# r9y9/deepvoice3_pytorch

Measured on NVIDIA H100. Metric: mel-frames/sec training step (B=16,T_mel=800), higher is better.
Workload: dtype f32 via split 16-bit pairs (fp16 pairs forward, bf16 pairs for gradients; 3 wgmma passes per product, fp32 accumulate)

## Files before the change

### deepvoice3_pytorch_b200/csrc/tc_gemm.cu

```cuda
#include "tc_common.cuh"
#include "../../include/dv3b200.h"

namespace dv3 {

using namespace tc;

constexpr int TC_CONV_THREADS = 512;
constexpr int TC_PRODUCER_REGS = 24;
constexpr int TC_CONSUMER_REGS = 176;
constexpr int TC_EPILOGUE_REGS = 136;
static_assert(TC_PRODUCER_REGS <= 65536 / TC_CONV_THREADS && TC_CONSUMER_REGS >= 65536 / TC_CONV_THREADS &&
              TC_EPILOGUE_REGS >= 65536 / TC_CONV_THREADS, "setmaxnreg direction of each warpgroup");
static_assert(128 * TC_PRODUCER_REGS + 256 * TC_CONSUMER_REGS + 128 * TC_EPILOGUE_REGS <= 65536, "register file");
constexpr int TC_WGRAD_THREADS = 288;
constexpr int MAX_TAPS_TC = 8;
constexpr int SMEM_LIMIT = 232448;
constexpr int RING_RESERVE = 32768;

enum { TC_GATED = 0, TC_CONV = 1 };

struct TcMaps { CUtensorMap a[2]; CUtensorMap b[2]; };

struct TcParams {
    int T, B;
    int Kc;
    int Nc;
    int rows_per_tap;
    int k, kb_n;
    int tap_off[MAX_TAPS_TC];
    const float* bias; const float* spk; const float* res;
    float* y; float* save_a; float* save_s;
    int gate_mode, residual;
    float* out; const float* e1; const float* e2; float alpha; int addmode, relu;
    float p_drop; const unsigned long long* seed_ptr; uint32_t salt;
    float gmain;
    int operand_bf16;
};

template <int BK> struct SwizzleOf;
template <> struct SwizzleOf<64> { static constexpr uint32_t layout = WG_SW128, sbo = 1024; };
template <> struct SwizzleOf<32> { static constexpr uint32_t layout = WG_SW64, sbo = 512; };

template <int BK>
__device__ __forceinline__ uint64_t make_desc(uint32_t saddr) {
    return make_wgmma_desc(saddr, 16, SwizzleOf<BK>::sbo, SwizzleOf<BK>::layout);
}

template <int NBOX, int BK, int BR, int NPL = 2>
struct TcCfg {
    static constexpr int TILE = 128 * BK * 2;
    static constexpr int TILE_B = BR * BK * 2;
    static constexpr int STAGE = NPL * (TILE + NBOX * TILE_B);
    static constexpr int NCOLS = BR * NBOX;
    static constexpr int ACC_PITCH = NCOLS + 1;
    static constexpr int ACC_TILE = 128 * ACC_PITCH * 4;
    static constexpr int STAGES_RAW = (SMEM_LIMIT - 2048 - RING_RESERVE - ACC_TILE) / STAGE;
    static constexpr int STAGES = STAGES_RAW > 6 ? 6 : STAGES_RAW;
    static constexpr int SMEM = STAGES * STAGE + ACC_TILE + 1024 + 512;
};
static_assert(TcCfg<2, 32, 64>::STAGES == 4, "gated forward: 4-stage ring");
static_assert(TcCfg<1, 32, 128>::STAGES == 4, "128-column conv: 4-stage ring");
static_assert(TcCfg<1, 64, 64>::STAGES == 3, "64-column conv at BK = 64: 3-stage ring");
static_assert(TcCfg<1, 32, 64>::STAGES == 6, "64-column conv at BK = 32: 6-stage ring");
static_assert(TcCfg<2, 64, 64, 1>::STAGES == 4, "single-pass gated forward: 4-stage ring");
static_assert(TcCfg<1, 64, 128, 1>::STAGES == 4, "single-pass 128-column conv at BK = 64: 4-stage ring");
static_assert(TcCfg<1, 32, 128, 1>::STAGES == 6, "single-pass 128-column conv at BK = 32: 6-stage ring");
static_assert(TcCfg<1, 64, 64, 1>::STAGES == 6, "single-pass 64-column conv at BK = 64: 6-stage ring");
static_assert(TcCfg<1, 32, 64, 1>::STAGES == 6, "single-pass 64-column conv at BK = 32: 6-stage ring");

template <int BR>
__device__ __forceinline__ void epilogue_gated(const TcParams& p, const float* arow, uint64_t* acc_empty, int a_row0,
                                               int a_z, int b_row0) {
    const int t = a_row0 + (threadIdx.x & 127), b = a_z, C = p.Nc;
    const bool tv = t < p.T;
    const float* __restrict__ bias = p.bias;
    const float* __restrict__ res = p.res;
    const float* __restrict__ spk = p.spk;
    float* __restrict__ yo = p.y;
    float* __restrict__ ao = p.save_a;
    float* __restrict__ so = p.save_s;
    const bool need_res = (p.gate_mode != 0) || p.residual;
    const size_t base = ((size_t)b * C + b_row0) * p.T + (tv ? t : 0);
#pragma unroll
    for (int c32 = 0; c32 < BR; c32 += 32) {
        float rr[32], sp[32];
        if (tv) {
            const size_t cb = base + (size_t)c32 * p.T;
#pragma unroll
            for (int i = 0; i < 32; ++i) rr[i] = need_res ? __ldg(&res[cb + (size_t)i * p.T]) : 0.f;
            if (spk) {
#pragma unroll
                for (int i = 0; i < 32; ++i) sp[i] = __ldg(&spk[cb + (size_t)i * p.T]);
            }
#pragma unroll
            for (int i = 0; i < 32; ++i) {
                const int c = b_row0 + c32 + i;
                const size_t idx = cb + (size_t)i * p.T;
                float va = arow[c32 + i];
                if (spk) va += sp[i];
                const float a = va + __ldg(&bias[c]);
                const float s = sigmoidf_(arow[BR + c32 + i] + __ldg(&bias[C + c]));
                float y;
                if (p.gate_mode == 0) {
                    y = a * s;
                    if (p.residual) y = (y + rr[i]) * 0.70710678118654752f;
                } else {
                    y = s * a + (1.f - s) * rr[i];
                }
                yo[idx] = y;
                if (ao) ao[idx] = a;
                if (so) so[idx] = s;
            }
        }
        if (c32 + 32 == BR) mbar_arrive(acc_empty);
    }
}

template <int NCOLS>
__device__ __forceinline__ void epilogue_conv(const TcParams& p, const float* arow, uint64_t* acc_empty, int a_row0,
                                              int a_z, int b_row0) {
    const int t = a_row0 + (threadIdx.x & 127), b = a_z;
    const bool tv = t < p.T;
    const DropCfg drop = make_drop(p.p_drop, p.seed_ptr, p.salt);
    const float* __restrict__ bias = p.bias;
    const float* __restrict__ e1 = p.e1;
    const float* __restrict__ e2 = p.e2;
    float* __restrict__ out = p.out;
#pragma unroll 1
    for (int c32 = 0; c32 < NCOLS; c32 += 32) {
        float v[32], x2[32];
        const int n0 = b_row0 + c32;
        const size_t cb = ((size_t)b * p.Nc + n0) * p.T + (tv ? t : 0);
        if (tv) {
#pragma unroll
            for (int i = 0; i < 32; ++i) {
                const bool ok = n0 + i < p.Nc;
                v[i] = (p.addmode != 0 && ok) ? __ldg(&e1[cb + (size_t)i * p.T]) : 0.f;
                x2[i] = (p.addmode == 2 && ok) ? __ldg(&e2[cb + (size_t)i * p.T]) : 0.f;
            }
#pragma unroll
            for (int i = 0; i < 32; ++i) {
                const int n = n0 + i;
                if (n < p.Nc) {
                    const size_t idx = cb + (size_t)i * p.T;
                    float g = arow[c32 + i] * drop_scale(drop, (uint32_t)idx);
                    if (bias) g += __ldg(&bias[n]);
                    if (p.addmode == 1) g += p.alpha * v[i];
                    else if (p.addmode == 2) g += v[i] * (1.f - x2[i]);
                    if (p.relu) g = fmaxf(g, 0.f);
                    out[idx] = g;
                }
            }
        }
        if (c32 + 32 == NCOLS) mbar_arrive(acc_empty);
    }
}

template <int MODE, int NBOX, int BR, int BK, bool BF16, int NPL>
__global__ void __launch_bounds__(TC_CONV_THREADS, 1)
tc_conv_kernel(const __grid_constant__ TcMaps maps, const __grid_constant__ TcParams p, int tiles_x, int tiles_y,
               int num_tiles) {
    pdl_trigger();
    static_assert(NPL == 1 || NPL == 2, "one or two operand planes");
    using Cfg = TcCfg<NBOX, BK, BR, NPL>;
    constexpr int TILE = Cfg::TILE, TILE_B = Cfg::TILE_B, STAGE = Cfg::STAGE, STAGES = Cfg::STAGES, NCOLS = Cfg::NCOLS;
    constexpr int B_OFF = NPL * TILE;
    constexpr int NR = NCOLS / 2;
    constexpr int A_HALF = 64 * BK * 2;
    static_assert(NCOLS <= 128, "main + cross accumulators must fit in the registers of a consumer thread");
    static_assert(STAGES >= 2, "pipeline needs at least two stages");
    extern __shared__ uint8_t smem_raw[];
    uint8_t* smem = reinterpret_cast<uint8_t*>((reinterpret_cast<uintptr_t>(smem_raw) + 1023) & ~(uintptr_t)1023);
    float* acc_tile = reinterpret_cast<float*>(smem + STAGES * STAGE);
    uint64_t* full = reinterpret_cast<uint64_t*>(smem + STAGES * STAGE + Cfg::ACC_TILE);
    uint64_t* empty = full + STAGES;
    uint64_t* acc_full = empty + STAGES;
    uint64_t* acc_empty = acc_full + 1;
    const int warp = threadIdx.x >> 5, lane = threadIdx.x & 31;
    const int n_iters = p.k * p.kb_n;

    if (threadIdx.x == 0) {
#pragma unroll
        for (int pl = 0; pl < NPL; ++pl) prefetch_tmap(&maps.a[pl]);
#pragma unroll
        for (int pl = 0; pl < NPL; ++pl) prefetch_tmap(&maps.b[pl]);
        for (int s = 0; s < STAGES; ++s) { mbar_init(&full[s], 1); mbar_init(&empty[s], 2); }
        mbar_init(acc_full, 256);
        mbar_init(acc_empty, 128);
        fence_barrier_init();
    }
    __syncthreads();
    pdl_wait();

    auto decode = [&](int tile, int& a_row0, int& a_z, int& b_row0, int& b_row1) {
        const int ty = tile % tiles_y, r = tile / tiles_y;
        const int tx = r % tiles_x;
        a_z = r / tiles_x;
        a_row0 = tx * 128;
        if (MODE == TC_GATED) { b_row0 = ty * BR; b_row1 = p.Nc + ty * BR; }
        else { b_row0 = ty * BR * NBOX; b_row1 = b_row0 + BR; }
    };

    if (warp >= 12) {
        setmaxnreg_inc<TC_EPILOGUE_REGS>();
        const float* arow = acc_tile + (threadIdx.x & 127) * Cfg::ACC_PITCH;
        int n = 0;
        for (int tile = blockIdx.x; tile < num_tiles; tile += gridDim.x, ++n) {
            int a_row0, a_z, b_row0, b_row1;
            decode(tile, a_row0, a_z, b_row0, b_row1);
            mbar_wait(acc_full, n & 1);
            if (MODE == TC_GATED) epilogue_gated<BR>(p, arow, acc_empty, a_row0, a_z, b_row0);
            else epilogue_conv<NCOLS>(p, arow, acc_empty, a_row0, a_z, b_row0);
        }
    } else if (warp >= 8) {
        setmaxnreg_dec<TC_PRODUCER_REGS>();
        if (warp == 8 && lane == 0) {
            int it = 0;
            for (int tile = blockIdx.x; tile < num_tiles; tile += gridDim.x) {
                int a_row0, a_z, b_row0, b_row1;
                decode(tile, a_row0, a_z, b_row0, b_row1);
                for (int kit = 0; kit < n_iters; ++kit, ++it) {
                    const int s = it % STAGES, ph = (it / STAGES) & 1;
                    mbar_wait(&empty[s], ph ^ 1);
                    uint8_t* st = smem + s * STAGE;
                    const int j = kit / p.kb_n, kb = kit - j * p.kb_n;
                    const int ax = kb * BK, ay = a_row0 + p.tap_off[j];
                    const int by0 = j * p.rows_per_tap + b_row0, by1 = j * p.rows_per_tap + b_row1;
                    mbar_arrive_expect_tx(&full[s], STAGE);
#pragma unroll
                    for (int pl = 0; pl < NPL; ++pl) {
                        tma_load_3d(st + pl * TILE, &maps.a[pl], &full[s], ax, ay, a_z);
                        uint8_t* bdst = st + B_OFF + pl * NBOX * TILE_B;
                        tma_load_3d(bdst, &maps.b[pl], &full[s], ax, by0, 0);
                        if (NBOX == 2) tma_load_3d(bdst + TILE_B, &maps.b[pl], &full[s], ax, by1, 0);
                    }
                }
            }
        }
    } else {
        setmaxnreg_inc<TC_CONSUMER_REGS>();
        const int wg = warp >> 2, wq = warp & 3;
        float acc[NR], xacc[NPL == 2 ? NR : 1];
        int it = 0, n = 0;
        for (int tile = blockIdx.x; tile < num_tiles; tile += gridDim.x, ++n) {
            int a_row0, a_z, b_row0, b_row1;
            decode(tile, a_row0, a_z, b_row0, b_row1);
#pragma unroll
            for (int i = 0; i < NR; ++i) {
                acc[i] = 0.f;
                if constexpr (NPL == 2) xacc[i] = 0.f;
            }
            for (int kit = 0; kit < n_iters; ++kit, ++it) {
                const int s = it % STAGES, ph = (it / STAGES) & 1;
                mbar_wait(&full[s], ph);
                const uint32_t sa = smem_u32(smem + s * STAGE) + wg * A_HALF;
                const uint32_t sb = smem_u32(smem + s * STAGE + B_OFF);
                wgmma_fence();
#pragma unroll
                for (int kk = 0; kk < BK / 16; ++kk) {
                    const uint32_t ko = kk * 32;
                    const uint64_t a0 = make_desc<BK>(sa + ko), b0 = make_desc<BK>(sb + ko);
                    wgmma_mma<NCOLS, 0, 0>(BF16, acc, a0, b0, 1);
                    if constexpr (NPL == 2) {
                        const uint64_t a1 = make_desc<BK>(sa + TILE + ko), b1 = make_desc<BK>(sb + NBOX * TILE_B + ko);
                        wgmma_mma<NCOLS, 0, 0>(BF16, xacc, a0, b1, 1);
                        wgmma_mma<NCOLS, 0, 0>(BF16, xacc, a1, b0, 1);
                    }
                }
                wgmma_commit();
                wgmma_wait<1>();
                if (kit > 0 && (threadIdx.x & 127) == 0) mbar_arrive(&empty[(it - 1) % STAGES]);
            }
            wgmma_wait<0>();
            if (n_iters > 0 && (threadIdx.x & 127) == 0) mbar_arrive(&empty[(it - 1) % STAGES]);
            mbar_wait(acc_empty, (n & 1) ^ 1);
#pragma unroll
            for (int i = 0; i < NR; ++i) {
                float* dst = &acc_tile[(64 * wg + frag_row(i, wq, lane)) * Cfg::ACC_PITCH + frag_col(i, lane)];
                if constexpr (NPL == 2) *dst = fmaf(xacc[i], LO_INV, acc[i] * p.gmain);
                else *dst = acc[i] * p.gmain;
            }
            mbar_arrive(acc_full);
        }
    }
}

struct TcMnParams {
    int T, B, Mw, Nw, k;
    int tap_off[MAX_TAPS_TC];
    int nsplit, batches_per_split, kb_n;
    float* dw; long long split_stride;
    int msplit; long long s_m, s_mh, s_n, s_j;
    float gcoef;
};

constexpr int WG_BOX = 64 * 32 * 2;
template <int NPL>
struct WgCfg {
    static constexpr int STAGE = NPL * (2 * WG_BOX + 2 * WG_BOX);
    static constexpr int STAGES = ((SMEM_LIMIT - 2048) / STAGE) > 6 ? 6 : ((SMEM_LIMIT - 2048) / STAGE);
    static constexpr int SMEM = STAGES * STAGE + 1024 + 512;
};
static_assert(WgCfg<2>::STAGES == 6 && WgCfg<1>::STAGES == 6, "weight gradient: 6-stage ring");

template <int NPL>
__global__ void __launch_bounds__(TC_WGRAD_THREADS, 1)
tc_wgrad_mn_kernel(const __grid_constant__ TcMaps maps, const __grid_constant__ TcMnParams p) {
    pdl_trigger();
    static_assert(NPL == 1 || NPL == 2, "one or two operand planes");
    constexpr int WG_STAGE = WgCfg<NPL>::STAGE, WG_STAGES = WgCfg<NPL>::STAGES;
    constexpr int A_PL = 2 * WG_BOX, B_PL = 2 * WG_BOX;
    constexpr uint32_t LBO = 4096, SBO = 1024;
    extern __shared__ uint8_t smem_raw[];
    uint8_t* smem = reinterpret_cast<uint8_t*>((reinterpret_cast<uintptr_t>(smem_raw) + 1023) & ~(uintptr_t)1023);
    uint64_t* full = reinterpret_cast<uint64_t*>(smem + WG_STAGES * WG_STAGE);
    uint64_t* empty = full + WG_STAGES;
    const int warp = threadIdx.x >> 5, lane = threadIdx.x & 31;

    const int wg_j = blockIdx.z % p.k, wg_split = blockIdx.z / p.k;
    const int m0 = blockIdx.y * 128, n0 = blockIdx.x * 128;
    const int b_beg = wg_split * p.batches_per_split;
    int b_end = b_beg + p.batches_per_split; if (b_end > p.B) b_end = p.B;
    const int n_iters = (b_end > b_beg ? b_end - b_beg : 0) * p.kb_n;

    if (threadIdx.x == 0) {
#pragma unroll
        for (int pl = 0; pl < NPL; ++pl) prefetch_tmap(&maps.a[pl]);
#pragma unroll
        for (int pl = 0; pl < NPL; ++pl) prefetch_tmap(&maps.b[pl]);
        for (int s = 0; s < WG_STAGES; ++s) { mbar_init(&full[s], 1); mbar_init(&empty[s], 2); }
        fence_barrier_init();
    }
    __syncthreads();
    pdl_wait();

    if (warp == 8) {
        if (lane == 0) {
            for (int it = 0; it < n_iters; ++it) {
                const int s = it % WG_STAGES, ph = (it / WG_STAGES) & 1;
                mbar_wait(&empty[s], ph ^ 1);
                uint8_t* st = smem + s * WG_STAGE;
                const int bi = it / p.kb_n, tc_ = it - bi * p.kb_n;
                const int b = b_beg + bi, t0 = tc_ * 32;
                mbar_arrive_expect_tx(&full[s], WG_STAGE);
#pragma unroll
                for (int pl = 0; pl < NPL; ++pl) {
#pragma unroll
                    for (int h = 0; h < 2; ++h)
                        tma_load_3d(st + pl * A_PL + h * WG_BOX, &maps.a[pl], &full[s], m0 + h * 64, t0, b);
#pragma unroll
                    for (int q = 0; q < 2; ++q)
                        tma_load_3d(st + NPL * A_PL + pl * B_PL + q * WG_BOX, &maps.b[pl], &full[s], n0 + q * 64,
                                    t0 + p.tap_off[wg_j], b);
                }
            }
        }
    } else {
        const int wg = warp >> 2, wq = warp & 3;
        float acc[NPL * 64];
#pragma unroll
        for (int i = 0; i < NPL * 64; ++i) acc[i] = 0.f;
        for (int it = 0; it < n_iters; ++it) {
            const int s = it % WG_STAGES, ph = (it / WG_STAGES) & 1;
            mbar_wait(&full[s], ph);
            const uint32_t sa = smem_u32(smem + s * WG_STAGE);
            wgmma_fence();
#pragma unroll
            for (int kk = 0; kk < 2; ++kk) {
                const uint32_t ko = kk * 16 * 128;
                const uint64_t a0 = make_wgmma_desc(sa + wg * WG_BOX + ko, LBO, SBO, WG_SW128);
                const uint64_t b0 = make_wgmma_desc(sa + NPL * A_PL + ko, LBO, SBO, WG_SW128);
                wgmma_mma<128, 1, 1>(true, acc, a0, b0, 1);
                if constexpr (NPL == 2) {
                    const uint64_t a1 = make_wgmma_desc(sa + A_PL + wg * WG_BOX + ko, LBO, SBO, WG_SW128);
                    const uint64_t b1 = make_wgmma_desc(sa + 2 * A_PL + B_PL + ko, LBO, SBO, WG_SW128);
                    wgmma_mma<128, 1, 1>(true, acc + 64, a0, b1, 1);
                    wgmma_mma<128, 1, 1>(true, acc + 64, a1, b0, 1);
                }
            }
            wgmma_commit();
            wgmma_wait<1>();
            if (it > 0 && (threadIdx.x & 127) == 0) mbar_arrive(&empty[(it - 1) % WG_STAGES]);
        }
        wgmma_wait<0>();
        float* __restrict__ out = p.dw + (size_t)wg_split * p.split_stride + (size_t)wg_j * p.s_j;
        const float gmain = 1.f + p.gcoef * (float)(2 * n_iters);
#pragma unroll
        for (int i = 0; i < 64; ++i) {
            const int m = m0 + 64 * wg + frag_row(i, wq, lane), n = n0 + frag_col(i, lane);
            if (m < p.Mw && n < p.Nw) {
                const size_t ma = (size_t)(m % p.msplit) * p.s_m + (size_t)(m / p.msplit) * p.s_mh;
                if constexpr (NPL == 2) out[ma + (size_t)n * p.s_n] = fmaf(acc[64 + i], LO_INV, acc[i] * gmain);
                else out[ma + (size_t)n * p.s_n] = acc[i] * gmain;
            }
        }
    }
}

typedef CUresult (*EncodeTiledFn)(CUtensorMap*, CUtensorMapDataType, cuuint32_t, void*, const cuuint64_t*,
                                  const cuuint64_t*, const cuuint32_t*, const cuuint32_t*, CUtensorMapInterleave,
                                  CUtensorMapSwizzle, CUtensorMapL2promotion, CUtensorMapFloatOOBfill);

static EncodeTiledFn encode_fn() {
    static const EncodeTiledFn fn = [] {
        void* f = nullptr;
        cudaDriverEntryPointQueryResult qres;
        cudaError_t e = cudaGetDriverEntryPoint("cuTensorMapEncodeTiled", &f, cudaEnableDefault, &qres);
        return (e == cudaSuccess) ? (EncodeTiledFn)f : (EncodeTiledFn) nullptr;
    }();
    return fn;
}

int encode_tmap_bf16_3d(CUtensorMap* map, const void* base, uint64_t d0, uint64_t d1, uint64_t d2,
                        uint64_t stride1_bytes, uint64_t stride2_bytes, uint32_t box0, uint32_t box1) {
    const EncodeTiledFn enc = encode_fn();
    if (!enc) { set_error("cuTensorMapEncodeTiled entry point unavailable"); return 1; }
    cuuint64_t dims[3] = {d0, d1, d2};
    cuuint64_t strides[2] = {stride1_bytes, stride2_bytes};
    cuuint32_t box[3] = {box0, box1, 1};
    cuuint32_t estr[3] = {1, 1, 1};
    const CUtensorMapSwizzle sw = box0 * 2 == 128 ? CU_TENSOR_MAP_SWIZZLE_128B : CU_TENSOR_MAP_SWIZZLE_64B;
    CUresult r = enc(map, CU_TENSOR_MAP_DATA_TYPE_BFLOAT16, 3, const_cast<void*>(base), dims, strides, box, estr,
                     CU_TENSOR_MAP_INTERLEAVE_NONE, sw, CU_TENSOR_MAP_L2_PROMOTION_L2_256B,
                     CU_TENSOR_MAP_FLOAT_OOB_FILL_NONE);
    if (r != CUDA_SUCCESS) {
        set_error("cuTensorMapEncodeTiled failed (%d): dims=(%llu,%llu,%llu) strides=(%llu,%llu) box=(%u,%u)", (int)r,
                  (unsigned long long)d0, (unsigned long long)d1, (unsigned long long)d2,
                  (unsigned long long)stride1_bytes, (unsigned long long)stride2_bytes, box0, box1);
        return 1;
    }
    return 0;
}

template <typename K>
static int ensure_smem(K kern, int bytes, const char* what) {
    cudaError_t e = cudaFuncSetAttribute(kern, cudaFuncAttributeMaxDynamicSharedMemorySize, bytes);
    if (e != cudaSuccess) { set_error("%s: cannot set %d B dynamic smem: %s", what, bytes, cudaGetErrorString(e)); return 1; }
    return 0;
}

template <int MODE, int NBOX, int BR, int BK, bool BF16, int NPL>
static int launch_conv_fmt(const TcMaps& maps, const TcParams& p, int tiles_x, int tiles_y, int batch, cudaStream_t st,
                       const char* what) {
    using Cfg = TcCfg<NBOX, BK, BR, NPL>;
    auto kern = tc_conv_kernel<MODE, NBOX, BR, BK, BF16, NPL>;
    static const int configured = ensure_smem(kern, Cfg::SMEM, what);
    if (configured) return 1;
    const int sms = config().sms;
    const int num_tiles = tiles_x * tiles_y * batch;
    const int grid = num_tiles < sms ? num_tiles : sms;
    cudaError_t e = launch_k(kern, dim3(grid), dim3(TC_CONV_THREADS), (size_t)Cfg::SMEM, st, maps, p, tiles_x, tiles_y,
                             num_tiles);
    if (e != cudaSuccess) { set_error("%s: launch failed: %s", what, cudaGetErrorString(e)); return 1; }
    return check_launch(what);
}

template <int MODE, int NBOX, int BR, int BK, int NPL = 2>
static int launch_conv(const TcMaps& maps, const TcParams& p, int tiles_x, int tiles_y, int batch, cudaStream_t st,
                       const char* what) {
    if (p.operand_bf16)
        return launch_conv_fmt<MODE, NBOX, BR, BK, true, NPL>(maps, p, tiles_x, tiles_y, batch, st, what);
    return launch_conv_fmt<MODE, NBOX, BR, BK, false, NPL>(maps, p, tiles_x, tiles_y, batch, st, what);
}

static void fill_taps_tc(int* tap_off, int k, int dilation, int causal, bool transpose) {
    const int padl = causal ? (k - 1) * dilation : (k - 1) / 2 * dilation;
    for (int j = 0; j < MAX_TAPS_TC; ++j)
        tap_off[j] = j < k ? (transpose ? (padl - j * dilation) : (j * dilation - padl)) : 0;
}

static inline const void* plane(const void* base, int pl, long long plane_elems) {
    return (const char*)base + (size_t)pl * plane_elems * 2;
}

}

using namespace dv3;

extern "C" {

int dv3_tc_supported(int B, int C, int T, int k) {
    return (C % 128 == 0) && T >= 1 && k >= 1 && k <= MAX_TAPS_TC && B >= 1 && B <= 65535;
}
int dv3_tc_conv_supported(int B, int Cin, int Cout, int T, int k) {
    return T >= 1 && k >= 1 && k <= MAX_TAPS_TC && B >= 1 && B <= 65535 && (k == 1 || Cout % 128 == 0) && Cin >= 8 &&
           Cout >= 1;
}

int dv3_tc_convblock_fwd(const void* xd, const void* w, int npl, const float* bias, const float* spk,
                         const float* res, float* y, float* save_a, float* save_s, int B, int C, int T, int k,
                         int dilation, int causal, int mode, int residual, const void* fuse, void* stream) {
    DV3_REQUIRE(dv3_tc_supported(B, C, T, k), "tc_convblock_fwd: unsupported shape B=%d C=%d T=%d k=%d", B, C, T, k);
    DV3_REQUIRE(npl == 1 || npl == 2, "tc_convblock_fwd: npl must be 1 or 2");
    DV3_REQUIRE(fuse == nullptr, "tc_convblock_fwd: fuse must be NULL");
    TcMaps maps;
    const int t_tiles = (T + 127) / 128;
    const int BK = npl == 2 ? 32 : 64;
    for (int pl = 0; pl < npl; ++pl) {
        if (encode_tmap_bf16_3d(&maps.a[pl], plane(xd, pl, (long long)B * T * C), C, T, B, (uint64_t)C * 2,
                                (uint64_t)T * C * 2, BK, 128)) return 1;
        if (encode_tmap_bf16_3d(&maps.b[pl], plane(w, pl, (long long)k * 2 * C * C), C, (uint64_t)k * 2 * C, 1,
                                (uint64_t)C * 2, (uint64_t)k * 2 * C * C * 2, BK, 64)) return 1;
    }
    TcParams p = {};
    p.T = T; p.B = B; p.Kc = C; p.Nc = C; p.rows_per_tap = 2 * C; p.k = k; p.kb_n = C / BK;
    fill_taps_tc(p.tap_off, k, dilation, causal, false);
    p.bias = bias; p.spk = spk; p.res = res; p.y = y; p.save_a = save_a; p.save_s = save_s;
    p.gate_mode = mode; p.residual = residual;
    p.gmain = 1.f + config().tc_gamma * (float)(p.k * p.kb_n * (BK / 16));
    p.operand_bf16 = 0;
    cudaStream_t st = (cudaStream_t)stream;
    if (npl == 1) return launch_conv<TC_GATED, 2, 64, 64, 1>(maps, p, t_tiles, C / 64, B, st, "tc_convblock_fwd");
    return launch_conv<TC_GATED, 2, 64, 32>(maps, p, t_tiles, C / 64, B, st, "tc_convblock_fwd");
}

int dv3_tc_conv(const void* a, const void* w, int npl, float* out, int B, int Kc, int Nc, int T, int k, int dilation,
                int causal, int transpose_taps, const float* bias, int relu, float p_drop,
                const unsigned long long* seed_ptr, unsigned salt, int addmode, const float* e1, const float* e2,
                float alpha, const void* fuse, void* stream) {
    DV3_REQUIRE(k >= 1 && k <= MAX_TAPS_TC && (k == 1 || Nc % 128 == 0) && B <= 65535,
                "tc_conv: unsupported shape B=%d Kc=%d Nc=%d T=%d k=%d", B, Kc, Nc, T, k);
    DV3_REQUIRE(npl == 1 || npl == 2, "tc_conv: npl must be 1 or 2");
    DV3_REQUIRE(fuse == nullptr, "tc_conv: fuse must be NULL");
    const int Kp = (Kc + 7) / 8 * 8;
    const int t_tiles = (T + 127) / 128;
    cudaStream_t st = (cudaStream_t)stream;
    const long long tiles128 = (long long)t_tiles * ((Nc + 127) / 128) * B;
    const bool narrow = Nc > 64 && (k == 1 || Nc % 64 == 0) && tiles128 < 100;
    const bool k64 = Kc % 64 == 0;
    const int bk = ((narrow || npl == 1) && k64) ? 64 : 32, br = narrow ? 64 : 128;
    TcMaps maps;
    for (int pl = 0; pl < npl; ++pl) {
        if (encode_tmap_bf16_3d(&maps.a[pl], plane(a, pl, (long long)B * T * Kp), Kc, T, B, (uint64_t)Kp * 2,
                                (uint64_t)T * Kp * 2, bk, 128)) return 1;
        if (encode_tmap_bf16_3d(&maps.b[pl], plane(w, pl, (long long)k * Nc * Kp), Kc, (uint64_t)k * Nc, 1,
                                (uint64_t)Kp * 2, (uint64_t)k * Nc * Kp * 2, bk, br)) return 1;
    }
    TcParams p = {};
    p.T = T; p.B = B; p.Kc = Kc; p.Nc = Nc; p.rows_per_tap = Nc; p.k = k; p.kb_n = (Kc + bk - 1) / bk;
    fill_taps_tc(p.tap_off, k, dilation, causal, transpose_taps != 0);
    p.out = out; p.bias = bias; p.relu = relu; p.e1 = e1; p.e2 = e2; p.alpha = alpha; p.addmode = addmode;
    p.p_drop = p_drop; p.seed_ptr = seed_ptr; p.salt = salt;
    p.gmain = 1.f + config().tc_gamma * (float)(p.k * p.kb_n * (bk / 16));
    p.operand_bf16 = transpose_taps ? 1 : 0;
    const int tiles_y = (Nc + br - 1) / br;
    if (npl == 1) {
        if (narrow) {
            if (k64) return launch_conv<TC_CONV, 1, 64, 64, 1>(maps, p, t_tiles, tiles_y, B, st, "tc_conv(64)");
            return launch_conv<TC_CONV, 1, 64, 32, 1>(maps, p, t_tiles, tiles_y, B, st, "tc_conv(64,bk32)");
        }
        if (k64) return launch_conv<TC_CONV, 1, 128, 64, 1>(maps, p, t_tiles, tiles_y, B, st, "tc_conv(128,bk64)");
        return launch_conv<TC_CONV, 1, 128, 32, 1>(maps, p, t_tiles, tiles_y, B, st, "tc_conv(128)");
    }
    if (narrow) {
        if (k64) return launch_conv<TC_CONV, 1, 64, 64>(maps, p, t_tiles, tiles_y, B, st, "tc_conv(64)");
        return launch_conv<TC_CONV, 1, 64, 32>(maps, p, t_tiles, tiles_y, B, st, "tc_conv(64,bk32)");
    }
    return launch_conv<TC_CONV, 1, 128, 32>(maps, p, t_tiles, tiles_y, B, st, "tc_conv(128)");
}

int dv3_tc_wgrad_nsplit(int B, int Mw, int Nw, int T, int k) {
    const int tiles = ((Mw + 127) / 128) * ((Nw + 127) / 128) * k;
    const int kb_n = (T + 31) / 32, sms = config().sms;
    int best = 1;
    for (int target = 2 * sms; target >= sms; target -= sms) {
        int want = (target + tiles - 1) / tiles;
        if (want > B) want = B;
        if (want < 1) want = 1;
        const int bps = (B + want - 1) / want;
        best = (B + bps - 1) / bps;
        if (bps * kb_n >= 64) break;
    }
    return best;
}

int dv3_tc_wgrad_mn_npl(const void* dy, const void* xd, int npl, float* dw_partials, long long split_stride, int B,
                        int Mw, int Nw, int T, int k, int dilation, int causal, int msplit, long long s_m,
                        long long s_mh, long long s_n, long long s_j, void* stream) {
    DV3_REQUIRE(k >= 1 && k <= MAX_TAPS_TC && B <= 65535, "tc_wgrad_mn: unsupported shape k=%d", k);
    DV3_REQUIRE(npl == 1 || npl == 2, "tc_wgrad_mn: npl must be 1 or 2");
    const int Mp = (Mw + 7) / 8 * 8, Np = (Nw + 7) / 8 * 8;
    TcMaps maps;
    for (int pl = 0; pl < npl; ++pl) {
        if (encode_tmap_bf16_3d(&maps.a[pl], plane(dy, pl, (long long)B * T * Mp), Mw, T, B, (uint64_t)Mp * 2,
                                (uint64_t)T * Mp * 2, 64, 32)) return 1;
        if (encode_tmap_bf16_3d(&maps.b[pl], plane(xd, pl, (long long)B * T * Np), Nw, T, B, (uint64_t)Np * 2,
                                (uint64_t)T * Np * 2, 64, 32)) return 1;
    }
    TcMnParams p = {};
    p.T = T; p.B = B; p.Mw = Mw; p.Nw = Nw; p.k = k; p.kb_n = (T + 31) / 32;
    fill_taps_tc(p.tap_off, k, dilation, causal, false);
    p.nsplit = dv3_tc_wgrad_nsplit(B, Mw, Nw, T, k);
    p.batches_per_split = (B + p.nsplit - 1) / p.nsplit;
    p.dw = dw_partials; p.split_stride = split_stride;
    p.msplit = msplit; p.s_m = s_m; p.s_mh = s_mh; p.s_n = s_n; p.s_j = s_j;
    p.gcoef = config().tc_gamma;
    const dim3 grid((Nw + 127) / 128, (Mw + 127) / 128, p.nsplit * k);
    cudaStream_t st = (cudaStream_t)stream;
    cudaError_t e;
    if (npl == 1) {
        static const int configured = ensure_smem(tc_wgrad_mn_kernel<1>, WgCfg<1>::SMEM, "tc_wgrad_mn");
        if (configured) return 1;
        e = launch_k(tc_wgrad_mn_kernel<1>, grid, dim3(TC_WGRAD_THREADS), (size_t)WgCfg<1>::SMEM, st, maps, p);
    } else {
        static const int configured = ensure_smem(tc_wgrad_mn_kernel<2>, WgCfg<2>::SMEM, "tc_wgrad_mn");
        if (configured) return 1;
        e = launch_k(tc_wgrad_mn_kernel<2>, grid, dim3(TC_WGRAD_THREADS), (size_t)WgCfg<2>::SMEM, st, maps, p);
    }
    if (e != cudaSuccess) { set_error("tc_wgrad_mn: launch failed: %s", cudaGetErrorString(e)); return 1; }
    return check_launch("tc_wgrad_mn");
}

int dv3_tc_wgrad_mn(const void* dy, const void* xd, float* dw_partials, long long split_stride, int B, int Mw,
                    int Nw, int T, int k, int dilation, int causal, int msplit, long long s_m, long long s_mh,
                    long long s_n, long long s_j, void* stream) {
    return dv3_tc_wgrad_mn_npl(dy, xd, 2, dw_partials, split_stride, B, Mw, Nw, T, k, dilation, causal, msplit, s_m,
                               s_mh, s_n, s_j, stream);
}

}
```

Before: 1.441 million.

## Share last-tile epilogue across consumer warpgroups and widen smem ring stages

Removes the smem ring reserve and caps stages by stage size, which gives the 64-column BK=64 conv a 4-stage ring instead of 3. For conv mode, the epilogue of each CTA's final tile is split into thirds: the two consumer warpgroups, idle once their mainloop ends, each store one third next to the epilogue warpgroup, shortening the tail. It also adds optional timing stamps that are compiled only under a define. The cost is extra consumer work at the end and a tighter smem budget.

```diff
diff --git a/deepvoice3_pytorch_b200/csrc/tc_gemm.cu b/deepvoice3_pytorch_b200/csrc/tc_gemm.cu
--- a/deepvoice3_pytorch_b200/csrc/tc_gemm.cu
+++ b/deepvoice3_pytorch_b200/csrc/tc_gemm.cu
@@ -15,9 +15,36 @@
 constexpr int TC_WGRAD_THREADS = 288;
 constexpr int MAX_TAPS_TC = 8;
 constexpr int SMEM_LIMIT = 232448;
-constexpr int RING_RESERVE = 32768;
 
 enum { TC_GATED = 0, TC_CONV = 1 };
+
+enum {
+    TS_NS,
+    TS_CLK,
+    TS_C_FULL,
+    TS_C_MMA,
+    TS_C_DRAIN,
+    TS_C_ACC_EMPTY,
+    TS_C_STORE,
+    TS_P_EMPTY,
+    TS_E_ACC_FULL,
+    TS_E_WORK,
+    TS_TILES,
+    TS_GRID,
+    TS_SLOTS = 16
+};
+#ifdef DV3_TC_STAMPS
+constexpr int TC_STAMP_CTAS = 1024;
+__device__ unsigned long long g_tc_stamps[TC_STAMP_CTAS][TS_SLOTS];
+__device__ __forceinline__ unsigned long long globaltimer_ns() {
+    unsigned long long t;
+    asm volatile("mov.u64 %0, %globaltimer;" : "=l"(t));
+    return t;
+}
+#define TC_STAMP(...) __VA_ARGS__
+#else
+#define TC_STAMP(...)
+#endif
 
 struct TcMaps { CUtensorMap a[2]; CUtensorMap b[2]; };
 
@@ -54,13 +81,14 @@
     static constexpr int NCOLS = BR * NBOX;
     static constexpr int ACC_PITCH = NCOLS + 1;
     static constexpr int ACC_TILE = 128 * ACC_PITCH * 4;
-    static constexpr int STAGES_RAW = (SMEM_LIMIT - 2048 - RING_RESERVE - ACC_TILE) / STAGE;
-    static constexpr int STAGES = STAGES_RAW > 6 ? 6 : STAGES_RAW;
+    static constexpr int STAGES_RAW = (SMEM_LIMIT - 2048 - ACC_TILE) / STAGE;
+    static constexpr int STAGES_MAX = STAGE >= 32768 ? 4 : 6;
+    static constexpr int STAGES = STAGES_RAW > STAGES_MAX ? STAGES_MAX : STAGES_RAW;
     static constexpr int SMEM = STAGES * STAGE + ACC_TILE + 1024 + 512;
 };
 static_assert(TcCfg<2, 32, 64>::STAGES == 4, "gated forward: 4-stage ring");
 static_assert(TcCfg<1, 32, 128>::STAGES == 4, "128-column conv: 4-stage ring");
-static_assert(TcCfg<1, 64, 64>::STAGES == 3, "64-column conv at BK = 64: 3-stage ring");
+static_assert(TcCfg<1, 64, 64>::STAGES == 4, "64-column conv at BK = 64: 4-stage ring");
 static_assert(TcCfg<1, 32, 64>::STAGES == 6, "64-column conv at BK = 32: 6-stage ring");
 static_assert(TcCfg<2, 64, 64, 1>::STAGES == 4, "single-pass gated forward: 4-stage ring");
 static_assert(TcCfg<1, 64, 128, 1>::STAGES == 4, "single-pass 128-column conv at BK = 64: 4-stage ring");
@@ -70,7 +98,7 @@
 
 template <int BR>
 __device__ __forceinline__ void epilogue_gated(const TcParams& p, const float* arow, uint64_t* acc_empty, int a_row0,
-                                               int a_z, int b_row0) {
+                                               int a_z, int b_row0, int c_lo = 0, int c_hi = BR) {
     const int t = a_row0 + (threadIdx.x & 127), b = a_z, C = p.Nc;
     const bool tv = t < p.T;
     const float* __restrict__ bias = p.bias;
@@ -82,7 +110,7 @@
     const bool need_res = (p.gate_mode != 0) || p.residual;
     const size_t base = ((size_t)b * C + b_row0) * p.T + (tv ? t : 0);
 #pragma unroll
-    for (int c32 = 0; c32 < BR; c32 += 32) {
+    for (int c32 = c_lo; c32 < c_hi; c32 += 32) {
         float rr[32], sp[32];
         if (tv) {
             const size_t cb = base + (size_t)c32 * p.T;
@@ -112,13 +140,13 @@
                 if (so) so[idx] = s;
             }
         }
-        if (c32 + 32 == BR) mbar_arrive(acc_empty);
+        if (c32 + 32 == c_hi && acc_empty) mbar_arrive(acc_empty);
     }
 }
 
 template <int NCOLS>
 __device__ __forceinline__ void epilogue_conv(const TcParams& p, const float* arow, uint64_t* acc_empty, int a_row0,
-                                              int a_z, int b_row0) {
+                                              int a_z, int b_row0, int c_lo = 0, int c_hi = NCOLS) {
     const int t = a_row0 + (threadIdx.x & 127), b = a_z;
     const bool tv = t < p.T;
     const DropCfg drop = make_drop(p.p_drop, p.seed_ptr, p.salt);
@@ -127,7 +155,7 @@
     const float* __restrict__ e2 = p.e2;
     float* __restrict__ out = p.out;
 #pragma unroll 1
-    for (int c32 = 0; c32 < NCOLS; c32 += 32) {
+    for (int c32 = c_lo; c32 < c_hi; c32 += 32) {
         float v[32], x2[32];
         const int n0 = b_row0 + c32;
         const size_t cb = ((size_t)b * p.Nc + n0) * p.T + (tv ? t : 0);
@@ -152,8 +180,14 @@
                 }
             }
         }
-        if (c32 + 32 == NCOLS) mbar_arrive(acc_empty);
-    }
+        if (c32 + 32 == c_hi && acc_empty) mbar_arrive(acc_empty);
+    }
+}
+
+__device__ __forceinline__ void split_last_tile(int cols, int part, int& lo, int& hi) {
+    const int chunks = cols / 32;
+    lo = 32 * (chunks * part / 3);
+    hi = 32 * (chunks * (part + 1) / 3);
 }
 
 template <int MODE, int NBOX, int BR, int BK, bool BF16, int NPL>
@@ -167,6 +201,8 @@
     constexpr int B_OFF = NPL * TILE;
     constexpr int NR = NCOLS / 2;
     constexpr int A_HALF = 64 * BK * 2;
+    constexpr int EPI_COLS = MODE == TC_GATED ? BR : NCOLS;
+    constexpr bool share_last = MODE == TC_CONV;
     static_assert(NCOLS <= 128, "main + cross accumulators must fit in the registers of a consumer thread");
     static_assert(STAGES >= 2, "pipeline needs at least two stages");
     extern __shared__ uint8_t smem_raw[];
@@ -204,24 +240,42 @@
     if (warp >= 12) {
         setmaxnreg_inc<TC_EPILOGUE_REGS>();
         const float* arow = acc_tile + (threadIdx.x & 127) * Cfg::ACC_PITCH;
+        TC_STAMP(long long e_wait = 0, e_work = 0;)
         int n = 0;
         for (int tile = blockIdx.x; tile < num_tiles; tile += gridDim.x, ++n) {
             int a_row0, a_z, b_row0, b_row1;
             decode(tile, a_row0, a_z, b_row0, b_row1);
+            TC_STAMP(const long long t0 = clock64();)
             mbar_wait(acc_full, n & 1);
-            if (MODE == TC_GATED) epilogue_gated<BR>(p, arow, acc_empty, a_row0, a_z, b_row0);
-            else epilogue_conv<NCOLS>(p, arow, acc_empty, a_row0, a_z, b_row0);
-        }
+            TC_STAMP(const long long t1 = clock64(); e_wait += t1 - t0;)
+            if (!share_last || tile + gridDim.x < num_tiles) {
+                if (MODE == TC_GATED) epilogue_gated<BR>(p, arow, acc_empty, a_row0, a_z, b_row0);
+                else epilogue_conv<NCOLS>(p, arow, acc_empty, a_row0, a_z, b_row0);
+            } else {
+                int lo, hi;
+                split_last_tile(EPI_COLS, 2, lo, hi);
+                if (MODE == TC_GATED) epilogue_gated<BR>(p, arow, acc_empty, a_row0, a_z, b_row0, lo, hi);
+                else epilogue_conv<NCOLS>(p, arow, acc_empty, a_row0, a_z, b_row0, lo, hi);
+            }
+            TC_STAMP(e_work += clock64() - t1;)
+        }
+        TC_STAMP(if (threadIdx.x == 384) {
+            g_tc_stamps[blockIdx.x][TS_E_ACC_FULL] = e_wait;
+            g_tc_stamps[blockIdx.x][TS_E_WORK] = e_work;
+        })
     } else if (warp >= 8) {
         setmaxnreg_dec<TC_PRODUCER_REGS>();
         if (warp == 8 && lane == 0) {
+            TC_STAMP(long long p_wait = 0;)
             int it = 0;
             for (int tile = blockIdx.x; tile < num_tiles; tile += gridDim.x) {
                 int a_row0, a_z, b_row0, b_row1;
                 decode(tile, a_row0, a_z, b_row0, b_row1);
                 for (int kit = 0; kit < n_iters; ++kit, ++it) {
                     const int s = it % STAGES, ph = (it / STAGES) & 1;
+                    TC_STAMP(const long long t0 = clock64();)
                     mbar_wait(&empty[s], ph ^ 1);
+                    TC_STAMP(p_wait += clock64() - t0;)
                     uint8_t* st = smem + s * STAGE;
                     const int j = kit / p.kb_n, kb = kit - j * p.kb_n;
                     const int ax = kb * BK, ay = a_row0 + p.tap_off[j];
@@ -236,11 +290,14 @@
                     }
                 }
             }
+            TC_STAMP(g_tc_stamps[blockIdx.x][TS_P_EMPTY] = p_wait;)
         }
     } else {
         setmaxnreg_inc<TC_CONSUMER_REGS>();
         const int wg = warp >> 2, wq = warp & 3;
         float acc[NR], xacc[NPL == 2 ? NR : 1];
+        TC_STAMP(long long c_full = 0, c_mma = 0, c_drain = 0, c_acc_empty = 0, c_store = 0;
+                 const unsigned long long g_begin = globaltimer_ns(); const long long k_begin = clock64();)
         int it = 0, n = 0;
         for (int tile = blockIdx.x; tile < num_tiles; tile += gridDim.x, ++n) {
             int a_row0, a_z, b_row0, b_row1;
@@ -252,7 +309,9 @@
             }
             for (int kit = 0; kit < n_iters; ++kit, ++it) {
                 const int s = it % STAGES, ph = (it / STAGES) & 1;
+                TC_STAMP(const long long t0 = clock64();)
                 mbar_wait(&full[s], ph);
+                TC_STAMP(const long long t1 = clock64(); c_full += t1 - t0;)
                 const uint32_t sa = smem_u32(smem + s * STAGE) + wg * A_HALF;
                 const uint32_t sb = smem_u32(smem + s * STAGE + B_OFF);
                 wgmma_fence();
@@ -270,10 +329,14 @@
                 wgmma_commit();
                 wgmma_wait<1>();
                 if (kit > 0 && (threadIdx.x & 127) == 0) mbar_arrive(&empty[(it - 1) % STAGES]);
-            }
+                TC_STAMP(c_mma += clock64() - t1;)
+            }
+            TC_STAMP(const long long t2 = clock64();)
             wgmma_wait<0>();
             if (n_iters > 0 && (threadIdx.x & 127) == 0) mbar_arrive(&empty[(it - 1) % STAGES]);
+            TC_STAMP(const long long t3 = clock64(); c_drain += t3 - t2;)
             mbar_wait(acc_empty, (n & 1) ^ 1);
+            TC_STAMP(const long long t4 = clock64(); c_acc_empty += t4 - t3;)
 #pragma unroll
             for (int i = 0; i < NR; ++i) {
                 float* dst = &acc_tile[(64 * wg + frag_row(i, wq, lane)) * Cfg::ACC_PITCH + frag_col(i, lane)];
@@ -281,7 +344,26 @@
                 else *dst = acc[i] * p.gmain;
             }
             mbar_arrive(acc_full);
-        }
+            TC_STAMP(c_store += clock64() - t4;)
+        }
+        int lo, hi;
+        split_last_tile(EPI_COLS, wg, lo, hi);
+        if (share_last && n > 0 && lo < hi) {
+            int a_row0, a_z, b_row0, b_row1;
+            decode(blockIdx.x + (n - 1) * gridDim.x, a_row0, a_z, b_row0, b_row1);
+            mbar_wait(acc_full, (n - 1) & 1);
+            const float* arow = acc_tile + (threadIdx.x & 127) * Cfg::ACC_PITCH;
+            if (MODE == TC_GATED) epilogue_gated<BR>(p, arow, nullptr, a_row0, a_z, b_row0, lo, hi);
+            else epilogue_conv<NCOLS>(p, arow, nullptr, a_row0, a_z, b_row0, lo, hi);
+        }
+        TC_STAMP(if (threadIdx.x == 0) {
+            unsigned long long* row = g_tc_stamps[blockIdx.x];
+            row[TS_NS] = globaltimer_ns() - g_begin;
+            row[TS_CLK] = clock64() - k_begin;
+            row[TS_C_FULL] = c_full; row[TS_C_MMA] = c_mma; row[TS_C_DRAIN] = c_drain;
+            row[TS_C_ACC_EMPTY] = c_acc_empty; row[TS_C_STORE] = c_store;
+            row[TS_TILES] = n; row[TS_GRID] = gridDim.x;
+        })
     }
 }
 
@@ -618,4 +700,13 @@
                                s_mh, s_n, s_j, stream);
 }
 
-}
+#ifdef DV3_TC_STAMPS
+int dv3_tc_stamps_read(unsigned long long* host, int rows) {
+    DV3_REQUIRE(rows >= 1 && rows <= TC_STAMP_CTAS, "tc_stamps_read: rows=%d", rows);
+    cudaError_t e = cudaMemcpyFromSymbol(host, g_tc_stamps, (size_t)rows * TS_SLOTS * sizeof(unsigned long long));
+    if (e != cudaSuccess) { set_error("tc_stamps_read: %s", cudaGetErrorString(e)); return 1; }
+    return 0;
+}
+#endif
+
+}
```

Result: no change. 1.443 million, median of 6 (+0.1%).
